# RikVoorhaar/tt-sketch

Hardware: AMD Instinct MI355X
Metric: TT-cores sketched/sec (fp64) + achieved MFMA % for d=6 n=200 r=50 stream_sketch (higher is better)
Workload: dtype f64

## Files before the change

tt_sketch_amd/csrc/chain_fused.h:

```cpp
#pragma once
#include "skinny.h"

namespace ttsk {

struct ChainStep {
    const double *W[SK_MAXB];
    const double *X[SK_MAXB];
    double *T[SK_MAXB];
    const double *E;
    double *slab;
    int nb, wpp, n;
    int K1, A, A2, J;
    int64_t w_c;
    int64_t x_j, x_k, x_c;
    int64_t x_extent, t_extent;
    int AP, A2P;
    int ebase;
    int eunits;
    int xcd_map;
    int diag;
    long long *stamps;
};

constexpr int CF_MAX_DMA = 160;

__device__ __forceinline__ void cf_barrier()
{
    asm volatile("s_waitcnt lgkmcnt(0)\n\ts_barrier" ::: "memory");
}
#ifdef TTSK_LAB
#define CF_DIAG(bit) (a.diag & (bit))
#define CF_STAMP(i) do { if (a.stamps && blockIdx.x == 0 && lane == 0 && k - k_beg < 8) a.stamps[((k - k_beg) * 8 + w) * 8 + (i)] = __builtin_amdgcn_s_memtime(); } while (0)
#else
#define CF_DIAG(bit) 0
#define CF_STAMP(i) do { } while (0)
#endif
#define CF_BARRIER() do { if (!CF_DIAG(4)) cf_barrier(); } while (0)

template <int NQF, int STRQ, int NNF, int STRN, int D, bool WT, int OCC, int EBUF, int UNR = 5 * D>
__global__ __launch_bounds__(512, 2 * OCC) void chain_step_kernel(ChainStep a)
{
    extern __shared__ double cf_lds[];
    double *Wl = cf_lds;
    double *El = cf_lds + a.ebase;
    const int tid = threadIdx.x, lane = tid & 63, w = tid >> 6;
    const int x16 = lane & 15, kq = lane >> 4;
    int prob, g;
    if (a.xcd_map) {
        const int gpx = a.wpp >> 3, xcd = blockIdx.x & 7, j = blockIdx.x >> 3;
        g = xcd * gpx + j % gpx;
        prob = j / gpx;
    } else {
        prob = blockIdx.x / a.wpp;
        g = blockIdx.x - prob * a.wpp;
    }
    const int k_beg = (int)((int64_t)g * a.n / a.wpp), k_end = (int)((int64_t)(g + 1) * a.n / a.wpp);
    const int NW = (a.J + 15) >> 4;
    const int KB1 = ((a.K1 + 3) / 4 + UNR - 1) / UNR * UNR;
    const int AP = a.AP, A2P = a.A2P;

    {
        const double *Wp = uniform_ptr(a.W[prob]);
        const __amdgpu_buffer_rsrc_t rw = make_rsrc(Wp, ((int64_t)(a.K1 - 1) * a.w_c + a.A) * 8);
        const int total = 4 * KB1 * AP;
        constexpr int BATCH = 10;
        for (int e0 = tid; e0 < total; e0 += 512 * BATCH) {
            double v[BATCH];
#pragma unroll
            for (int u = 0; u < BATCH; ++u) {
                const int e = e0 + 512 * u;
                const int c = e / AP, col = e - c * AP;
                v[u] = ld8(rw, (e < total && c < a.K1 && col < a.A) ? (uint32_t)(((int64_t)c * a.w_c + col) * 8) : OOB_OFF, 0);
            }
#pragma unroll
            for (int u = 0; u < BATCH; ++u) {
                const int e = e0 + 512 * u;
                const int c = e / AP, col = e - c * AP;
                if (e < total) Wl[(c >> 1) * 2 * AP + 2 * col + (c & 1)] = v[u];
            }
        }
    }

    if (w == 7) {
        const int NI = CF_DIAG(2) ? 0 : a.eunits >> 6;
        const uint32_t inv = (uint32_t)(((1ull << 32) + (uint32_t)A2P - 1) / (uint32_t)A2P);
        const int64_t rowstride = (int64_t)a.n * a.A2;
        const int ebuf = a.eunits * 2;
        auto fill = [&](int k) {
            const double *Ek = a.E + (int64_t)k * a.A2;
            double *dst = El + (EBUF == 2 ? (k & 1) * ebuf : 0);
#pragma unroll 2
            for (int m = 0; m < NI; ++m) {
                const uint32_t U = 64u * (uint32_t)m + (uint32_t)lane;
                const uint32_t sec = (uint32_t)(((uint64_t)U * inv) >> 32), u = U - sec * (uint32_t)A2P;
                int row = (int)(2 * sec + (u & 1));
                row = row < a.A ? row : a.A - 1;
                int col = (int)(2 * (u >> 1));
                col = col + 1 < a.A2 ? col : 0;
                __builtin_amdgcn_global_load_lds((const __attribute__((address_space(1))) void *)(Ek + row * rowstride + col),
                                                 (__attribute__((address_space(3))) void *)(dst + m * 128), 16, 0, 0);
            }
        };
        __syncthreads();
        if constexpr (EBUF == 2) {
            if (k_beg < k_end) fill(k_beg);
            for (int k = k_beg; k < k_end; ++k) {
                asm volatile("s_waitcnt vmcnt(0)" ::: "memory");
                CF_STAMP(1);
                CF_BARRIER();
                CF_STAMP(2);
                if (k + 1 < k_end) fill(k + 1);
                CF_STAMP(3);
                CF_BARRIER();
                CF_STAMP(4);
            }
        } else {
            for (int k = k_beg; k < k_end; ++k) {
                CF_STAMP(0);
                fill(k);
                asm volatile("s_waitcnt vmcnt(0)" ::: "memory");
                CF_STAMP(1);
                CF_BARRIER();
                CF_STAMP(2);
                CF_STAMP(3);
                CF_BARRIER();
                CF_STAMP(4);
            }
        }
        return;
    }
    __syncthreads();
    if (w >= NW) return;

    const int j0 = 16 * w;
    const bool jok = j0 + x16 < a.J;
    const uint32_t xlane = !CF_DIAG(1) ? (uint32_t)(((int64_t)(j0 + x16) * a.x_j + (int64_t)kq * a.x_c) * 8) : OOB_OFF;
    const __amdgpu_buffer_rsrc_t rx = make_rsrc(uniform_ptr(a.X[prob]), a.x_extent * 8);
    const uint32_t xstep = __builtin_amdgcn_readfirstlane((uint32_t)(4 * a.x_c * 8));
    const uint32_t kstep = __builtin_amdgcn_readfirstlane((uint32_t)(a.x_k * 8));
    static_assert(UNR % D == 0, "the unrolled body must keep the ring slots static");
    const int ITER = KB1 / UNR;
    auto xload = [&](uint32_t so) -> double { return ld8(rx, xlane, __builtin_amdgcn_readfirstlane(so)); };
    double ring[D];
#pragma unroll
    for (int d = 0; d < D; ++d) ring[d] = xload((uint32_t)k_beg * kstep + (uint32_t)d * xstep);

    v4d acc2[NNF ? NNF : 1];
    double acc2s[STRN ? STRN : 1];
#pragma unroll
    for (int p = 0; p < NNF; ++p)
#pragma unroll
        for (int t = 0; t < 4; ++t) acc2[p][t] = 0.0;
#pragma unroll
    for (int q = 0; q < STRN; ++q) acc2s[q] = 0.0;

    const int wl_lane = (kq >> 1) * 2 * AP + 2 * x16 + (kq & 1);
    const int ws_lane = (kq >> 1) * 2 * AP + 2 * (16 * NQF + (x16 & 3)) + (kq & 1);
    const int el_lane = (kq >> 1) * 2 * A2P + 4 * (x16 >> 1) + 2 * (kq & 1) + (x16 & 1);
    const int es_col = 16 * NNF + (x16 & 3);
    const int es_lane = (kq >> 1) * 2 * A2P + 2 * (kq & 1);

    __amdgpu_buffer_rsrc_t rt;
    if constexpr (WT) rt = make_rsrc(uniform_ptr(a.T[prob]), a.t_extent * 8);

    for (int k = k_beg; k < k_end; ++k) {
        v4d acc1[NQF ? NQF : 1];
        double acc1s[STRQ ? STRQ : 1];
#pragma unroll
        for (int p = 0; p < NQF; ++p)
#pragma unroll
            for (int t = 0; t < 4; ++t) acc1[p][t] = 0.0;
#pragma unroll
        for (int q = 0; q < STRQ; ++q) acc1s[q] = 0.0;

        CF_STAMP(0);
        double af[NQF ? NQF : 1], sf[STRQ ? STRQ : 1];
        auto wfetch = [&](const double *wrun, int u, double (&f)[NQF ? NQF : 1], double (&g)[STRQ ? STRQ : 1]) {
#pragma unroll
            for (int p = 0; p < NQF; ++p) f[p] = LDS_UNPAIRED(wrun[wl_lane + u * 4 * AP + 32 * p]);
#pragma unroll
            for (int q = 0; q < STRQ; ++q) g[q] = wrun[ws_lane + u * 4 * AP + 8 * q];
        };
        wfetch(Wl, 0, af, sf);
        uint32_t so = (uint32_t)k * kstep + (uint32_t)D * xstep;
        auto kblock = [&](const double *wrun, int u, bool wrap) {
            const int d = u % D;
            double afn[NQF ? NQF : 1], sfn[STRQ ? STRQ : 1];
            wfetch(wrun, u + 1, afn, sfn);
            const double bf = ring[d];
#pragma unroll
            for (int p = 0; p < NQF; ++p) acc1[p] = mfma16(af[p], bf, acc1[p]);
#pragma unroll
            for (int q = 0; q < STRQ; ++q) acc1s[q] = mfma4(sf[q], bf, acc1s[q]);
            if (wrap) so = (uint32_t)(k + 1) * kstep;
            ring[d] = xload(so);
            so += xstep;
#pragma unroll
            for (int p = 0; p < NQF; ++p) af[p] = afn[p];
#pragma unroll
            for (int q = 0; q < STRQ; ++q) sf[q] = sfn[q];
        };
        for (int it = 0; it < ITER; ++it) {
            const double *wrun = Wl + it * UNR * 4 * AP;
            const bool last = it == ITER - 1;
#pragma unroll
            for (int u = 0; u < UNR; ++u) kblock(wrun, u, last && u + D == UNR);
        }
        if constexpr (WT) {
            const int64_t nJ = (int64_t)a.n * a.J;
            const uint32_t tl = jok ? (uint32_t)(((int64_t)kq * nJ + (int64_t)k * a.J + j0 + x16) * 8) : OOB_OFF;
#pragma unroll
            for (int p = 0; p < NQF; ++p)
#pragma unroll
                for (int t = 0; t < 4; ++t)
                    st8(rt, (jok && 16 * p + 4 * t + kq < a.A) ? tl + (uint32_t)((16 * p + 4 * t) * nJ * 8) : OOB_OFF, acc1[p][t]);
#pragma unroll
            for (int q = 0; q < STRQ; ++q)
                st8(rt, (jok && 16 * NQF + 4 * q + kq < a.A) ? tl + (uint32_t)((16 * NQF + 4 * q) * nJ * 8) : OOB_OFF, acc1s[q]);
        }
        CF_STAMP(1);
        CF_BARRIER();
        CF_STAMP(2);

        {
            const double *eb = El + (EBUF == 2 ? (k & 1) * a.eunits * 2 : 0);
            double bf[NNF ? NNF : 1], bs[STRN ? STRN : 1];
            int el0 = el_lane, es0 = es_lane + 4 * (es_col >> 1) + (es_col & 1);
            asm volatile("" : "+v"(el0), "+v"(es0));
            auto efetch = [&](int kap, double (&f)[NNF ? NNF : 1], double (&g)[STRN ? STRN : 1]) {
#pragma unroll
                for (int nn = 0; nn < NNF; ++nn) f[nn] = LDS_UNPAIRED(eb[el0 + kap * 4 * A2P + 32 * nn]);
#pragma unroll
                for (int q = 0; q < STRN; ++q) g[q] = eb[es0 + kap * 4 * A2P + 8 * q];
            };
            double bf2[NNF ? NNF : 1], bs2[STRN ? STRN : 1];
            efetch(0, bf, bs);
            constexpr int KB2C = 4 * NQF + STRQ;
#pragma unroll
            for (int kap = 0; kap < KB2C; ++kap) {
                const int p = kap >> 2, t = kap & 3;
                const double af2 = p < NQF ? acc1[p < NQF ? p : 0][t] : acc1s[t < STRQ ? t : 0];
                if (kap & 1) {
                    if (kap + 1 < KB2C) efetch(kap + 1, bf, bs);
                    __builtin_amdgcn_sched_barrier(0);
#pragma unroll
                    for (int nn = 0; nn < NNF; ++nn) acc2[nn] = mfma16(af2, bf2[nn], acc2[nn]);
#pragma unroll
                    for (int q = 0; q < STRN; ++q) acc2s[q] = mfma4(af2, bs2[q], acc2s[q]);
                } else {
                    if (kap + 1 < KB2C) efetch(kap + 1, bf2, bs2);
                    __builtin_amdgcn_sched_barrier(0);
#pragma unroll
                    for (int nn = 0; nn < NNF; ++nn) acc2[nn] = mfma16(af2, bf[nn], acc2[nn]);
#pragma unroll
                    for (int q = 0; q < STRN; ++q) acc2s[q] = mfma4(af2, bs[q], acc2s[q]);
                }
            }
        }
        CF_STAMP(3);
        CF_BARRIER();
        CF_STAMP(4);
    }

    double *slab = a.slab + ((int64_t)prob * a.wpp + g) * a.J * a.A2;
#pragma unroll
    for (int nn = 0; nn < NNF; ++nn)
#pragma unroll
        for (int t = 0; t < 4; ++t) {
            const int j = j0 + 4 * t + kq, col = 16 * nn + x16;
            if (j < a.J && col < a.A2) slab[(int64_t)j * a.A2 + col] = acc2[nn][t];
        }
#pragma unroll
    for (int q = 0; q < STRN; ++q) {
        const int j = j0 + 4 * ((lane >> 2) & 3) + kq, col = 16 * NNF + 4 * q + (lane & 3);
        if (j < a.J && col < a.A2) slab[(int64_t)j * a.A2 + col] = acc2s[q];
    }
}

struct ChainStepArgs {
    int nb, n, K1, A, A2, J;
    const double *const *W;
    int64_t w_c;
    const double *const *X;
    int64_t x_j, x_k, x_c, x_extent;
    const double *E;
    double *const *T;
    double *const *Out;
};
int chain_fused_try(const ChainStepArgs &c, int stream, hipStream_t st, bool force = false);

}
```

tt_sketch_amd/csrc/chain_fused.hip:

```cpp
#include <cstdlib>
#include "chain_fused.h"

namespace ttsk {

int launch_chain_step_a(const ChainStep &a, int nf, int str, bool wt, int ebuf, int unr, size_t lds, int grid, hipStream_t st);
int launch_chain_step_b(const ChainStep &a, int nf, int str, bool wt, int ebuf, int unr, size_t lds, int grid, hipStream_t st);
int launch_chain_step_c(const ChainStep &a, int nf, int str, bool wt, int ebuf, int unr, size_t lds, int grid, hipStream_t st);
int launch_chain_step_d(const ChainStep &a, int nf, int str, bool wt, int ebuf, int unr, size_t lds, int grid, hipStream_t st);
int launch_chain_step_e(const ChainStep &a, int nf, int str, bool wt, int ebuf, int unr, size_t lds, int grid, hipStream_t st);

static int launch_chain_step(const ChainStep &a, int nf, int str, bool wt, int ebuf, int unr, size_t lds, int grid, hipStream_t st)
{
    if (nf <= 2) return launch_chain_step_a(a, nf, str, wt, ebuf, unr, lds, grid, st);
    if (nf <= 4) return launch_chain_step_b(a, nf, str, wt, ebuf, unr, lds, grid, st);
    if (nf == 5) return launch_chain_step_c(a, nf, str, wt, ebuf, unr, lds, grid, st);
    if (nf == 6) return launch_chain_step_d(a, nf, str, wt, ebuf, unr, lds, grid, st);
    return launch_chain_step_e(a, nf, str, wt, ebuf, unr, lds, grid, st);
}

static int cf_num_cu()
{
    static int n = [] {
        int dev = 0, v = 0;
        if (hipGetDevice(&dev) != hipSuccess) return 256;
        if (hipDeviceGetAttribute(&v, hipDeviceAttributeMultiprocessorCount, dev) != hipSuccess || v <= 0) return 256;
        return v;
    }();
    return n;
}

static void tile_split(int r, int &nf, int &str)
{
    const int rem = r % 16;
    nf = r / 16;
    if (rem == 0) str = 0;
    else if (rem <= 4) str = 1;
    else if (rem <= 8) str = 2;
    else { nf += 1; str = 0; }
}

// ... 19 lines not shown
    a.AP = 16 * nq + 4 * sq;
    a.A2P = c.A2;
    if (a.AP < 4 * KB2) return 0;
    const int64_t wl = (int64_t)4 * KB1 * a.AP;
    a.ebase = (int)((wl + 1) & ~(int64_t)1);
    const int64_t units = (int64_t)2 * KB2 * a.A2P;
    a.eunits = (int)cdiv(units, 64) * 64;
    if (a.eunits / 64 > CF_MAX_DMA) return 0;
    const int ebuf = nq <= 4 ? 2 : 1;
    const size_t lds = ((size_t)a.ebase + (size_t)a.eunits * 2 * ebuf) * 8;
    if (lds > 160 * 1024) return 0;
#ifdef TTSK_LAB
    { static int dg = [] { const char *e = getenv("TTSK_CF_DIAG"); return e ? atoi(e) : 0; }(); a.diag = dg; }
#endif
    if ((c.x_extent + c.x_k + 132 * c.x_c) * 8 >= (1ll << 32) - 64) return 0;
    if ((int64_t)c.A * c.n * c.A2 * 8 >= (1ll << 32) - 64) return 0;
    const bool wt = c.T != nullptr;
    a.t_extent = (int64_t)c.A * c.n * c.J;
    if (wt && (a.t_extent + (int64_t)16 * c.n * c.J) * 8 >= (1ll << 32) - 64) return 0;
    const int cus = cf_num_cu();
    int wpp = cus / c.nb > 0 ? cus / c.nb : 1;
    if (wpp > c.n) wpp = c.n;
    a.wpp = wpp;
    a.xcd_map = (wpp % 8 == 0 && wpp >= 8) ? 1 : 0;
    for (int b = 0; b < c.nb; ++b) {
        if ((uintptr_t)c.X[b] & 7) return 0;
        a.W[b] = c.W[b];
        a.X[b] = c.X[b];
        a.T[b] = wt ? c.T[b] : nullptr;
    }
    const int64_t nslab = (int64_t)c.nb * wpp;
    a.slab = (double *)scratch(stream, SCRATCH_GEMM, (size_t)nslab * c.J * c.A2 * 8 + 64);
    if (!a.slab) return TTSK_ERR_HIP;
    const bool prof = prof_on();
    if (prof) prof_open(st, 2.0 * c.nb * (double)c.n * c.J * ((double)c.K1 * c.A + (double)c.A * c.A2), 6,
                        nq * 100 + sq * 10 + (wt ? 1 : 0), unr == 25, false);
#ifdef TTSK_LAB
    static int stamps_on = [] { const char *e = getenv("TTSK_CF_STAMPS"); return e ? atoi(e) : 0; }();
#else
    constexpr int stamps_on = 0;
#endif
    long long *stamps_dev = nullptr;
    if (stamps_on) {
        if (hipMalloc(&stamps_dev, 8 * 8 * 8 * 8) != hipSuccess) return TTSK_ERR_HIP;
        (void)hipMemset(stamps_dev, 0, 8 * 8 * 8 * 8);
        a.stamps = stamps_dev;
    }
    int rc = launch_chain_step(a, nq, sq, wt, ebuf, unr, lds, (int)nslab, st);
    if (stamps_on) {
        long long h[8 * 8 * 8];
        (void)hipStreamSynchronize(st);
        (void)hipMemcpy(h, stamps_dev, sizeof(h), hipMemcpyDeviceToHost);
        (void)hipFree(stamps_dev);
        long long t0 = 0;
        for (int i = 0; i < 8 * 8 * 8; ++i) if (h[i] && (!t0 || h[i] < t0)) t0 = h[i];
        fprintf(stderr, "[cf stamps] workgroup 0: cycles since its first stamp; per slice, wave: start | endA | afterB1 | endB | afterB2\n");
        for (int sl = 0; sl < 4; ++sl)
            for (int w = 0; w < 8; ++w) {
                const long long *r = h + (sl * 8 + w) * 8;
                if (!r[1] && !r[4]) continue;
                fprintf(stderr, "  slice %d wave %d: %8lld %8lld %8lld %8lld %8lld\n", sl, w, r[0] ? r[0] - t0 : -1, r[1] - t0, r[2] - t0,
                        r[3] - t0, r[4] - t0);
            }
    }
    if (rc == TTSK_OK) {
        ReduceOut ro{};
        for (int b = 0; b < c.nb; ++b) ro.C[b] = c.Out[b];
        rc = launch_r_reduce(st, a.slab, wpp, c.J, c.A2, 1, (int64_t)c.J, ro, c.nb, (int64_t)c.A2, (int64_t)1, 1.0, 0);
    }
    if (prof) prof_close(st);
    return rc == TTSK_OK ? 1 : (rc == 1 ? 0 : rc);
}

}

using namespace ttsk;

extern "C" int ttsk_chain_step(int nb, int n, int K1, int A, int A2, int J, const double *const *W, int64_t w_c,
                               const double *const *X, int64_t x_j, int64_t x_k, int64_t x_c, int64_t x_extent,
                               const double *E, double *const *T, double *const *Out, int stream)
{
    TTSK_STREAM(st, stream);
// ... 11 lines not shown
```

tt_sketch_amd/csrc/chain_fused_ia.hip:

```cpp
#include "chain_fused_inst.h"

namespace ttsk {

int launch_chain_step_a(const ChainStep &a, int nf, int str, bool wt, int ebuf, int unr, size_t lds, int grid, hipStream_t st)
{
    TTSK_CF_CASE(1, 0, 2)
    TTSK_CF_CASE(1, 1, 2)
    TTSK_CF_CASE(1, 2, 2)
    TTSK_CF_CASE(2, 0, 2)
    TTSK_CF_CASE(2, 1, 2)
    TTSK_CF_CASE(2, 2, 2)
    return 1;
}

}
```

tt_sketch_amd/csrc/chain_fused_ib.hip:

```cpp
#include "chain_fused_inst.h"

namespace ttsk {

int launch_chain_step_b(const ChainStep &a, int nf, int str, bool wt, int ebuf, int unr, size_t lds, int grid, hipStream_t st)
{
    TTSK_CF_CASE(3, 0, 2)
    TTSK_CF_CASE(3, 1, 2)
    TTSK_CF_CASE(3, 2, 2)
    TTSK_CF_CASE(4, 0, 2)
    TTSK_CF_CASE(4, 1, 2)
    TTSK_CF_CASE(4, 2, 2)
    return 1;
}

}
```

tt_sketch_amd/csrc/chain_fused_ic.hip:

```cpp
#include "chain_fused_inst.h"

namespace ttsk {

int launch_chain_step_c(const ChainStep &a, int nf, int str, bool wt, int ebuf, int unr, size_t lds, int grid, hipStream_t st)
{
    TTSK_CF_CASE(5, 0, 1)
    TTSK_CF_CASE(5, 1, 1)
    TTSK_CF_CASE(5, 2, 1)
    return 1;
}

}
```

tt_sketch_amd/csrc/chain_fused_id.hip:

```cpp
#include "chain_fused_inst.h"

namespace ttsk {

int launch_chain_step_d(const ChainStep &a, int nf, int str, bool wt, int ebuf, int unr, size_t lds, int grid, hipStream_t st)
{
    TTSK_CF_CASE(6, 0, 1)
    TTSK_CF_CASE(6, 1, 1)
    TTSK_CF_CASE(6, 2, 1)
    return 1;
}

}
```

tt_sketch_amd/csrc/chain_fused_ie.hip:

```cpp
#include "chain_fused_inst.h"

namespace ttsk {

int launch_chain_step_e(const ChainStep &a, int nf, int str, bool wt, int ebuf, int unr, size_t lds, int grid, hipStream_t st)
{
    TTSK_CF_CASE(7, 0, 1)
    return 1;
}

}
```

tt_sketch_amd/csrc/chain_fused_inst.h:

```cpp
#pragma once
#include "chain_fused.h"

namespace ttsk {

#define TTSK_CF_KERN(NF, STR, WT, EBUF, UNR) chain_step_kernel<NF, STR, NF, STR, 5, WT, 1, EBUF, UNR>
#define TTSK_CF_CASE(NF, STR, EBUF)                                                                          \
    if (nf == NF && str == STR && ebuf == EBUF)                                                              \
        return launch(unr == 25 ? (wt ? TTSK_CF_KERN(NF, STR, true, EBUF, 25) : TTSK_CF_KERN(NF, STR, false, EBUF, 25)) \
                                : (wt ? TTSK_CF_KERN(NF, STR, true, EBUF, 5) : TTSK_CF_KERN(NF, STR, false, EBUF, 5)),   \
                      grid, 512, lds, st, a);

}
```

Measured before the change: 55420.

## Deal chain-step tiles across 12 waves with split and narrow-row pieces

Adds a host-side planner that splits the J tiles into pieces (whole tiles, tiles cut along the A dimension into two halves, and a 4-row variant for narrow trailing tiles) and assigns them to up to 12 waves, greedily balancing MFMA cycles across the four SIMDs. The kernel gains a 12-wave instantiation that dispatches each wave to its piece. Split halves combine their partial slab results through a block barrier and a read-modify-write. Spare waves are marked as load slots. The aim is to remove SIMD imbalance when the tile count does not map evenly onto 4 SIMDs, at the cost of lower occupancy (launch bounds of 1 block), extra barriers and more register pressure.

```diff
diff --git a/tt_sketch_amd/csrc/chain_deal.h b/tt_sketch_amd/csrc/chain_deal.h
--- /dev/null
+++ b/tt_sketch_amd/csrc/chain_deal.h
@@ -0,0 +1,99 @@
+#pragma once
+
+namespace ttsk {
+
+constexpr int CD_WAVES = 12;
+constexpr int CD_MAXPIECE = CD_WAVES - 1;
+constexpr int CD_NQF_MIN = 2, CD_KB2_MAX = 25;
+enum ChainPieceKind { CD_NONE = 0, CD_WHOLE = 1, CD_FIRST = 2, CD_REST = 3, CD_ROWS4 = 4 };
+
+constexpr int cd_cut(int nqf) { return nqf - (nqf + 1) / 3; }
+
+struct ChainPiece {
+    int tile;
+    int q0, nq;
+    int kind;
+    int slot;
+    long long cycles;
+};
+
+struct ChainDeal {
+    int waves;
+    int npieces;
+    ChainPiece piece[CD_MAXPIECE];
+    long long simd[4];
+    double useful;
+    double cap() const
+    {
+        long long m = simd[0];
+        for (int s = 1; s < 4; ++s) m = simd[s] > m ? simd[s] : m;
+        return m > 0 ? useful / (4.0 * (double)m) : 0.0;
+    }
+};
+
+inline ChainDeal chain_deal(int J, int A, int A2, int NQF, int STRQ, int NNF, int STRN, int kb1, bool cut = true)
+{
+    (void)A; (void)A2;
+    const long long colB = 64ll * NNF + 16ll * STRN;
+    auto cost = [&](int nfull, int nstrip) {
+        return (long long)kb1 * (64ll * nfull + 16ll * nstrip) + (long long)(4 * nfull + nstrip) * colB;
+    };
+    const long long cW = cost(NQF, STRQ);
+    const long long cR = 16ll * (NQF + STRQ) * (kb1 + 4 * NNF + STRN);
+    const int H = cd_cut(NQF);
+    const int NW = (J + 15) / 16;
+    const bool narrow = J % 16 >= 1 && J % 16 <= 4;
+
+    ChainDeal best{};
+    best.waves = 8;
+    best.npieces = NW;
+    for (int w = 0; w < NW; ++w) {
+        best.piece[w] = ChainPiece{w, 0, NQF + STRQ, CD_WHOLE, w, cW};
+        best.simd[w & 3] += cW;
+    }
+    best.useful = (double)J / 16.0 * (double)cW;
+    if (!cut || NW <= 4 || NW > 7 || NQF < CD_NQF_MIN || 4 * NQF + STRQ > CD_KB2_MAX) return best;
+
+    long long best_max = 0;
+    for (int s = 0; s < 4; ++s) best_max = best.simd[s] > best_max ? best.simd[s] : best_max;
+    const int nfull = narrow ? NW - 1 : NW;
+    for (int ncut = 0; ncut <= nfull; ++ncut) {
+        if (nfull + ncut + (narrow ? 1 : 0) > CD_MAXPIECE) break;
+        if (ncut == 0 && !narrow) continue;
+        ChainDeal d{};
+        d.waves = CD_WAVES;
+        d.useful = best.useful;
+        int np = 0;
+        for (int t = 0; t < nfull - ncut; ++t) d.piece[np++] = ChainPiece{t, 0, NQF + STRQ, CD_WHOLE, -1, cW};
+        for (int t = nfull - ncut; t < nfull; ++t) d.piece[np++] = ChainPiece{t, 0, H, CD_FIRST, -1, cost(H, 0)};
+        for (int t = nfull - ncut; t < nfull; ++t)
+            d.piece[np++] = ChainPiece{t, H, NQF - H + STRQ, CD_REST, -1, cost(NQF - H, STRQ)};
+        if (narrow) d.piece[np++] = ChainPiece{NW - 1, 0, NQF + STRQ, CD_ROWS4, -1, cR};
+        d.npieces = np;
+        for (int i = 1; i < np; ++i)
+            for (int j = i; j > 0 && d.piece[j].cycles > d.piece[j - 1].cycles; --j) {
+                const ChainPiece tmp = d.piece[j];
+                d.piece[j] = d.piece[j - 1];
+                d.piece[j - 1] = tmp;
+            }
+        int used[4] = {0, 0, 0, 0};
+        const int room[4] = {3, 3, 3, 2};
+        for (int i = 0; i < np; ++i) {
+            int s = -1;
+            for (int c = 0; c < 4; ++c)
+                if (used[c] < room[c] && (s < 0 || d.simd[c] < d.simd[s])) s = c;
+            d.piece[i].slot = s + 4 * used[s];
+            used[s] += 1;
+            d.simd[s] += d.piece[i].cycles;
+        }
+        long long m = 0;
+        for (int s = 0; s < 4; ++s) m = d.simd[s] > m ? d.simd[s] : m;
+        if (m < best_max) {
+            best_max = m;
+            best = d;
+        }
+    }
+    return best;
+}
+
+}
diff --git a/tt_sketch_amd/csrc/chain_fused.h b/tt_sketch_amd/csrc/chain_fused.h
--- a/tt_sketch_amd/csrc/chain_fused.h
+++ b/tt_sketch_amd/csrc/chain_fused.h
@@ -1,4 +1,5 @@
 #pragma once
+#include "chain_deal.h"
 #include "skinny.h"
 
 namespace ttsk {
@@ -18,6 +19,8 @@
     int ebase;
     int eunits;
     int xcd_map;
+    unsigned int piece[CD_WAVES];
+    int nload;
     int diag;
     long long *stamps;
 };
@@ -30,21 +33,290 @@
 }
 #ifdef TTSK_LAB
 #define CF_DIAG(bit) (a.diag & (bit))
-#define CF_STAMP(i) do { if (a.stamps && blockIdx.x == 0 && lane == 0 && k - k_beg < 8) a.stamps[((k - k_beg) * 8 + w) * 8 + (i)] = __builtin_amdgcn_s_memtime(); } while (0)
+#define CF_STAMP(i) do { if (a.stamps && blockIdx.x == 0 && lane == 0 && k - k_beg < 8) a.stamps[((k - k_beg) * CD_WAVES + w) * 8 + (i)] = __builtin_amdgcn_s_memtime(); } while (0)
 #else
 #define CF_DIAG(bit) 0
 #define CF_STAMP(i) do { } while (0)
 #endif
 #define CF_BARRIER() do { if (!CF_DIAG(4)) cf_barrier(); } while (0)
 
-template <int NQF, int STRQ, int NNF, int STRN, int D, bool WT, int OCC, int EBUF, int UNR = 5 * D>
-__global__ __launch_bounds__(512, 2 * OCC) void chain_step_kernel(ChainStep a)
+template <int NQF, int STRQ, int NNF, int STRN, int D, bool WT, int EBUF, int UNR, int KIND, int APC = 0>
+__device__ __forceinline__ void cf_piece(const ChainStep &a, const double *Wl, const double *El, int tile, int q0, int prob,
+                                         int g, int k_beg, int k_end, int KB1, int w, int lane)
+{
+    const int x16 = lane & 15, kq = lane >> 4;
+    const int AP = APC ? APC : a.AP, A2P = a.A2P;
+    const int j0 = 16 * tile;
+    const bool jok = j0 + x16 < a.J;
+    const uint32_t xlane = !CF_DIAG(1) ? (uint32_t)(((int64_t)(j0 + x16) * a.x_j + (int64_t)kq * a.x_c) * 8) : OOB_OFF;
+    const __amdgpu_buffer_rsrc_t rx = make_rsrc(uniform_ptr(a.X[prob]), a.x_extent * 8);
+    const uint32_t xstep = __builtin_amdgcn_readfirstlane((uint32_t)(4 * a.x_c * 8));
+    const uint32_t kstep = __builtin_amdgcn_readfirstlane((uint32_t)(a.x_k * 8));
+    static_assert(UNR % D == 0, "the unrolled body must keep the ring slots static");
+    const int ITER = KB1 / UNR;
+    auto xload = [&](uint32_t so) -> double { return ld8(rx, xlane, __builtin_amdgcn_readfirstlane(so)); };
+    double ring[D];
+#pragma unroll
+    for (int d = 0; d < D; ++d) ring[d] = xload((uint32_t)k_beg * kstep + (uint32_t)d * xstep);
+
+    v4d acc2[NNF ? NNF : 1];
+    double acc2s[STRN ? STRN : 1];
+#pragma unroll
+    for (int p = 0; p < NNF; ++p)
+#pragma unroll
+        for (int t = 0; t < 4; ++t) acc2[p][t] = 0.0;
+#pragma unroll
+    for (int q = 0; q < STRN; ++q) acc2s[q] = 0.0;
+
+    const int wl_lane = (kq >> 1) * 2 * AP + 2 * (16 * q0 + x16) + (kq & 1);
+    const int ws_lane = (kq >> 1) * 2 * AP + 2 * (16 * (q0 + NQF) + (x16 & 3)) + (kq & 1);
+    const int el_lane = (kq >> 1) * 2 * A2P + 4 * (x16 >> 1) + 2 * (kq & 1) + (x16 & 1);
+    const int es_col = 16 * NNF + (x16 & 3);
+    const int es_lane = (kq >> 1) * 2 * A2P + 2 * (kq & 1);
+
+    __amdgpu_buffer_rsrc_t rt;
+    if constexpr (WT) rt = make_rsrc(uniform_ptr(a.T[prob]), a.t_extent * 8);
+
+    for (int k = k_beg; k < k_end; ++k) {
+        v4d acc1[NQF ? NQF : 1];
+        double acc1s[STRQ ? STRQ : 1];
+#pragma unroll
+        for (int p = 0; p < NQF; ++p)
+#pragma unroll
+            for (int t = 0; t < 4; ++t) acc1[p][t] = 0.0;
+#pragma unroll
+        for (int q = 0; q < STRQ; ++q) acc1s[q] = 0.0;
+
+        CF_STAMP(0);
+        double af[NQF ? NQF : 1], sf[STRQ ? STRQ : 1];
+        auto wfetch = [&](const double *wrun, int u, double (&f)[NQF ? NQF : 1], double (&g)[STRQ ? STRQ : 1]) {
+#pragma unroll
+            for (int p = 0; p < NQF; ++p) f[p] = LDS_UNPAIRED(wrun[wl_lane + u * 4 * AP + 32 * p]);
+#pragma unroll
+            for (int q = 0; q < STRQ; ++q) g[q] = wrun[ws_lane + u * 4 * AP + 8 * q];
+        };
+        wfetch(Wl, 0, af, sf);
+        uint32_t so = (uint32_t)k * kstep + (uint32_t)D * xstep;
+        auto kblock = [&](const double *wrun, int u, bool wrap) {
+            const int d = u % D;
+            double afn[NQF ? NQF : 1], sfn[STRQ ? STRQ : 1];
+            wfetch(wrun, u + 1, afn, sfn);
+            const double bf = ring[d];
+#pragma unroll
+            for (int p = 0; p < NQF; ++p) acc1[p] = mfma16(af[p], bf, acc1[p]);
+#pragma unroll
+            for (int q = 0; q < STRQ; ++q) acc1s[q] = mfma4(sf[q], bf, acc1s[q]);
+            if (wrap) so = (uint32_t)(k + 1) * kstep;
+            ring[d] = xload(so);
+            so += xstep;
+#pragma unroll
+            for (int p = 0; p < NQF; ++p) af[p] = afn[p];
+#pragma unroll
+            for (int q = 0; q < STRQ; ++q) sf[q] = sfn[q];
+        };
+        for (int it = 0; it < ITER; ++it) {
+            const double *wrun = Wl + it * UNR * 4 * AP;
+            const bool last = it == ITER - 1;
+#pragma unroll
+            for (int u = 0; u < UNR; ++u) kblock(wrun, u, last && u + D == UNR);
+        }
+        if constexpr (WT) {
+            const int64_t nJ = (int64_t)a.n * a.J;
+            const int a0 = 16 * q0;
+            const uint32_t tl = jok ? (uint32_t)(((int64_t)(a0 + kq) * nJ + (int64_t)k * a.J + j0 + x16) * 8) : OOB_OFF;
+#pragma unroll
+            for (int p = 0; p < NQF; ++p)
+#pragma unroll
+                for (int t = 0; t < 4; ++t)
+                    st8(rt, (jok && a0 + 16 * p + 4 * t + kq < a.A) ? tl + (uint32_t)((16 * p + 4 * t) * nJ * 8) : OOB_OFF, acc1[p][t]);
+#pragma unroll
+            for (int q = 0; q < STRQ; ++q)
+                st8(rt, (jok && a0 + 16 * NQF + 4 * q + kq < a.A) ? tl + (uint32_t)((16 * NQF + 4 * q) * nJ * 8) : OOB_OFF, acc1s[q]);
+        }
+        CF_STAMP(1);
+        CF_BARRIER();
+        CF_STAMP(2);
+
+        {
+            const double *eb = El + (EBUF == 2 ? (k & 1) * a.eunits * 2 : 0) + q0 * 16 * A2P;
+            double bf[NNF ? NNF : 1], bs[STRN ? STRN : 1];
+            int el0 = el_lane, es0 = es_lane + 4 * (es_col >> 1) + (es_col & 1);
+            asm volatile("" : "+v"(el0), "+v"(es0));
+            auto efetch = [&](int kap, double (&f)[NNF ? NNF : 1], double (&g)[STRN ? STRN : 1]) {
+#pragma unroll
+                for (int nn = 0; nn < NNF; ++nn) f[nn] = LDS_UNPAIRED(eb[el0 + kap * 4 * A2P + 32 * nn]);
+#pragma unroll
+                for (int q = 0; q < STRN; ++q) g[q] = eb[es0 + kap * 4 * A2P + 8 * q];
+            };
+            double bf2[NNF ? NNF : 1], bs2[STRN ? STRN : 1];
+            efetch(0, bf, bs);
+            constexpr int KB2C = 4 * NQF + STRQ;
+#pragma unroll
+            for (int kap = 0; kap < KB2C; ++kap) {
+                const int p = kap >> 2, t = kap & 3;
+                const double af2 = p < NQF ? acc1[p < NQF ? p : 0][t] : acc1s[t < STRQ ? t : 0];
+                if (kap & 1) {
+                    if (kap + 1 < KB2C) efetch(kap + 1, bf, bs);
+                    __builtin_amdgcn_sched_barrier(0);
+#pragma unroll
+                    for (int nn = 0; nn < NNF; ++nn) acc2[nn] = mfma16(af2, bf2[nn], acc2[nn]);
+#pragma unroll
+                    for (int q = 0; q < STRN; ++q) acc2s[q] = mfma4(af2, bs2[q], acc2s[q]);
+                } else {
+                    if (kap + 1 < KB2C) efetch(kap + 1, bf2, bs2);
+                    __builtin_amdgcn_sched_barrier(0);
+#pragma unroll
+                    for (int nn = 0; nn < NNF; ++nn) acc2[nn] = mfma16(af2, bf[nn], acc2[nn]);
+#pragma unroll
+                    for (int q = 0; q < STRN; ++q) acc2s[q] = mfma4(af2, bs[q], acc2s[q]);
+                }
+            }
+        }
+        CF_STAMP(3);
+        CF_BARRIER();
+        CF_STAMP(4);
+    }
+
+    double *slab = a.slab + ((int64_t)prob * a.wpp + g) * a.J * a.A2;
+    if constexpr (KIND == CD_FIRST) __syncthreads();
+    int ln = lane;
+    if constexpr (APC != 0) asm volatile("v_mbcnt_lo_u32_b32 %0, -1, 0\n\tv_mbcnt_hi_u32_b32 %0, -1, %0" : "=v"(ln));
+    const int sx = ln & 15, sk = ln >> 4;
+#pragma unroll
+    for (int nn = 0; nn < NNF; ++nn)
+#pragma unroll
+        for (int t = 0; t < 4; ++t) {
+            const int j = j0 + 4 * t + sk, col = 16 * nn + sx;
+            if (j < a.J && col < a.A2) {
+                double *p = slab + (int64_t)j * a.A2 + col;
+                *p = KIND == CD_FIRST ? acc2[nn][t] + *p : acc2[nn][t];
+            }
+        }
+#pragma unroll
+    for (int q = 0; q < STRN; ++q) {
+        const int j = j0 + 4 * ((ln >> 2) & 3) + sk, col = 16 * NNF + 4 * q + (ln & 3);
+        if (j < a.J && col < a.A2) {
+            double *p = slab + (int64_t)j * a.A2 + col;
+            *p = KIND == CD_FIRST ? acc2s[q] + *p : acc2s[q];
+        }
+    }
+    if constexpr (KIND == CD_REST) {
+        __threadfence_block();
+        __syncthreads();
+    }
+}
+
+template <int NQF, int STRQ, int NNF, int STRN, int D, bool WT, int EBUF, int UNR, int APC>
+__device__ __forceinline__ void cf_rows4(const ChainStep &a, const double *Wl, const double *El, int tile, int prob, int g,
+                                         int k_beg, int k_end, int KB1, int w, int lane)
+{
+    constexpr int NC = 4 * NNF + STRN;
+    __builtin_amdgcn_s_setprio(2);
+    const int x16 = lane & 15, kq = lane >> 4, n4 = x16 & 3, beta = x16 >> 2;
+    constexpr int AP = APC;
+    const int A2P = a.A2P;
+    const int j0 = 16 * tile;
+    const bool jok = j0 + n4 < a.J;
+    const uint32_t xlane = !CF_DIAG(1) ? (uint32_t)(((int64_t)(j0 + n4) * a.x_j + (int64_t)kq * a.x_c) * 8) : OOB_OFF;
+    const __amdgpu_buffer_rsrc_t rx = make_rsrc(uniform_ptr(a.X[prob]), a.x_extent * 8);
+    const uint32_t xstep = __builtin_amdgcn_readfirstlane((uint32_t)(4 * a.x_c * 8));
+    const uint32_t kstep = __builtin_amdgcn_readfirstlane((uint32_t)(a.x_k * 8));
+    const int ITER = KB1 / UNR;
+    auto xload = [&](uint32_t so) -> double { return ld8(rx, xlane, __builtin_amdgcn_readfirstlane(so)); };
+    double ring[D];
+#pragma unroll
+    for (int d = 0; d < D; ++d) ring[d] = xload((uint32_t)k_beg * kstep + (uint32_t)d * xstep);
+
+    double acc2[NC];
+#pragma unroll
+    for (int c = 0; c < NC; ++c) acc2[c] = 0.0;
+
+    const int wl_lane = (kq >> 1) * 2 * AP + 2 * x16 + (kq & 1);
+    const int ws_lane = (kq >> 1) * 2 * AP + 2 * (16 * NQF + n4) + (kq & 1);
+    const int el_lane = (2 * beta + (kq >> 1)) * 2 * A2P + 4 * (n4 >> 1) + 2 * (kq & 1) + (n4 & 1);
+    const int es_lane = (kq >> 1) * 2 * A2P + 4 * (n4 >> 1) + 2 * (kq & 1) + (n4 & 1);
+
+    __amdgpu_buffer_rsrc_t rt;
+    if constexpr (WT) rt = make_rsrc(uniform_ptr(a.T[prob]), a.t_extent * 8);
+
+    for (int k = k_beg; k < k_end; ++k) {
+        double acc1[NQF], acc1s[STRQ ? STRQ : 1];
+#pragma unroll
+        for (int p = 0; p < NQF; ++p) acc1[p] = 0.0;
+#pragma unroll
+        for (int q = 0; q < STRQ; ++q) acc1s[q] = 0.0;
+        CF_STAMP(0);
+        uint32_t so = (uint32_t)k * kstep + (uint32_t)D * xstep;
+        for (int it = 0; it < ITER; ++it) {
+            const double *wrun = Wl + it * UNR * 4 * AP;
+            const bool last = it == ITER - 1;
+#pragma unroll
+            for (int u = 0; u < UNR; ++u) {
+                const int d = u % D;
+                const double bf = ring[d];
+#pragma unroll
+                for (int p = 0; p < NQF; ++p) acc1[p] = mfma4(LDS_UNPAIRED(wrun[wl_lane + u * 4 * AP + 32 * p]), bf, acc1[p]);
+#pragma unroll
+                for (int q = 0; q < STRQ; ++q) acc1s[q] = mfma4(wrun[ws_lane + u * 4 * AP + 8 * q], bf, acc1s[q]);
+                if (last && u + D == UNR) so = (uint32_t)(k + 1) * kstep;
+                ring[d] = xload(so);
+                so += xstep;
+            }
+        }
+        if constexpr (WT) {
+            const int64_t nJ = (int64_t)a.n * a.J;
+            const uint32_t tl = (uint32_t)(((int64_t)kq * nJ + (int64_t)k * a.J + j0 + n4) * 8);
+#pragma unroll
+            for (int p = 0; p < NQF; ++p)
+                st8(rt, (jok && 16 * p + 4 * beta + kq < a.A) ? tl + (uint32_t)((16 * p + 4 * beta) * nJ * 8) : OOB_OFF, acc1[p]);
+#pragma unroll
+            for (int q = 0; q < STRQ; ++q)
+                st8(rt, (jok && beta == 0 && 16 * NQF + 4 * q + kq < a.A) ? tl + (uint32_t)((16 * NQF + 4 * q) * nJ * 8) : OOB_OFF,
+                    acc1s[q]);
+        }
+        CF_STAMP(1);
+        CF_BARRIER();
+        CF_STAMP(2);
+        {
+            const double *eb = El + (EBUF == 2 ? (k & 1) * a.eunits * 2 : 0);
+            int el0 = el_lane, es0 = es_lane;
+            asm volatile("" : "+v"(el0), "+v"(es0));
+#pragma unroll
+            for (int p = 0; p < NQF; ++p)
+#pragma unroll
+                for (int c = 0; c < NC; ++c) acc2[c] = mfma4(acc1[p], eb[el0 + p * 16 * A2P + 8 * c], acc2[c]);
+#pragma unroll
+            for (int q = 0; q < STRQ; ++q)
+#pragma unroll
+                for (int c = 0; c < NC; ++c) {
+                    const double e = eb[es0 + (8 * NQF + 2 * q) * 2 * A2P + 8 * c];
+                    acc2[c] = mfma4(acc1s[q], beta == 0 ? e : 0.0, acc2[c]);
+                }
+        }
+        CF_STAMP(3);
+        CF_BARRIER();
+        CF_STAMP(4);
+    }
+
+    double *slab = a.slab + ((int64_t)prob * a.wpp + g) * a.J * a.A2;
+#pragma unroll
+    for (int c = 0; c < NC; ++c) {
+        double v = acc2[c];
+        v += __shfl_xor(v, 4);
+        v += __shfl_xor(v, 8);
+        const int j = j0 + kq, col = 4 * c + n4;
+        if (beta == 0 && j < a.J && col < a.A2) slab[(int64_t)j * a.A2 + col] = v;
+    }
+}
+
+template <int NQF, int STRQ, int NNF, int STRN, int D, bool WT, int OCC, int EBUF, int UNR = 5 * D, int NWV = 8>
+__global__ __launch_bounds__(64 * NWV, NWV == 8 ? 2 * OCC : 1) void chain_step_kernel(ChainStep a)
 {
     extern __shared__ double cf_lds[];
     double *Wl = cf_lds;
     double *El = cf_lds + a.ebase;
     const int tid = threadIdx.x, lane = tid & 63, w = tid >> 6;
-    const int x16 = lane & 15, kq = lane >> 4;
+    constexpr int NT = 64 * NWV;
     int prob, g;
     if (a.xcd_map) {
         const int gpx = a.wpp >> 3, xcd = blockIdx.x & 7, j = blockIdx.x >> 3;
@@ -55,7 +327,6 @@
         g = blockIdx.x - prob * a.wpp;
     }
     const int k_beg = (int)((int64_t)g * a.n / a.wpp), k_end = (int)((int64_t)(g + 1) * a.n / a.wpp);
-    const int NW = (a.J + 15) >> 4;
     const int KB1 = ((a.K1 + 3) / 4 + UNR - 1) / UNR * UNR;
     const int AP = a.AP, A2P = a.A2P;
 
@@ -64,24 +335,32 @@
         const __amdgpu_buffer_rsrc_t rw = make_rsrc(Wp, ((int64_t)(a.K1 - 1) * a.w_c + a.A) * 8);
         const int total = 4 * KB1 * AP;
         constexpr int BATCH = 10;
-        for (int e0 = tid; e0 < total; e0 += 512 * BATCH) {
+        for (int e0 = tid; e0 < total; e0 += NT * BATCH) {
             double v[BATCH];
 #pragma unroll
             for (int u = 0; u < BATCH; ++u) {
-                const int e = e0 + 512 * u;
+                const int e = e0 + NT * u;
                 const int c = e / AP, col = e - c * AP;
                 v[u] = ld8(rw, (e < total && c < a.K1 && col < a.A) ? (uint32_t)(((int64_t)c * a.w_c + col) * 8) : OOB_OFF, 0);
             }
 #pragma unroll
             for (int u = 0; u < BATCH; ++u) {
-                const int e = e0 + 512 * u;
+                const int e = e0 + NT * u;
                 const int c = e / AP, col = e - c * AP;
                 if (e < total) Wl[(c >> 1) * 2 * AP + 2 * col + (c & 1)] = v[u];
             }
         }
     }
 
-    if (w == 7) {
+    unsigned pc = 0;
+    int li = 0, nl = 1;
+    if constexpr (NWV != 8) {
+        pc = a.piece[__builtin_amdgcn_readfirstlane(w)];
+        li = __builtin_amdgcn_readfirstlane((pc >> 8) & 255);
+        nl = a.nload;
+    }
+    if (NWV == 8 ? w == 7 : __builtin_amdgcn_readfirstlane(pc >> 16) == CD_NONE) {
+        if constexpr (NWV != 8) __builtin_amdgcn_s_setprio(3);
         const int NI = CF_DIAG(2) ? 0 : a.eunits >> 6;
         const uint32_t inv = (uint32_t)(((1ull << 32) + (uint32_t)A2P - 1) / (uint32_t)A2P);
         const int64_t rowstride = (int64_t)a.n * a.A2;
@@ -90,7 +369,7 @@
             const double *Ek = a.E + (int64_t)k * a.A2;
             double *dst = El + (EBUF == 2 ? (k & 1) * ebuf : 0);
 #pragma unroll 2
-            for (int m = 0; m < NI; ++m) {
+            for (int m = li; m < NI; m += nl) {
                 const uint32_t U = 64u * (uint32_t)m + (uint32_t)lane;
                 const uint32_t sec = (uint32_t)(((uint64_t)U * inv) >> 32), u = U - sec * (uint32_t)A2P;
                 int row = (int)(2 * sec + (u & 1));
@@ -130,150 +409,20 @@
         return;
     }
     __syncthreads();
-    if (w >= NW) return;
-
-    const int j0 = 16 * w;
-    const bool jok = j0 + x16 < a.J;
-    const uint32_t xlane = !CF_DIAG(1) ? (uint32_t)(((int64_t)(j0 + x16) * a.x_j + (int64_t)kq * a.x_c) * 8) : OOB_OFF;
-    const __amdgpu_buffer_rsrc_t rx = make_rsrc(uniform_ptr(a.X[prob]), a.x_extent * 8);
-    const uint32_t xstep = __builtin_amdgcn_readfirstlane((uint32_t)(4 * a.x_c * 8));
-    const uint32_t kstep = __builtin_amdgcn_readfirstlane((uint32_t)(a.x_k * 8));
-    static_assert(UNR % D == 0, "the unrolled body must keep the ring slots static");
-    const int ITER = KB1 / UNR;
-    auto xload = [&](uint32_t so) -> double { return ld8(rx, xlane, __builtin_amdgcn_readfirstlane(so)); };
-    double ring[D];
-#pragma unroll
-    for (int d = 0; d < D; ++d) ring[d] = xload((uint32_t)k_beg * kstep + (uint32_t)d * xstep);
-
-    v4d acc2[NNF ? NNF : 1];
-    double acc2s[STRN ? STRN : 1];
-#pragma unroll
-    for (int p = 0; p < NNF; ++p)
-#pragma unroll
-        for (int t = 0; t < 4; ++t) acc2[p][t] = 0.0;
-#pragma unroll
-    for (int q = 0; q < STRN; ++q) acc2s[q] = 0.0;
-
-    const int wl_lane = (kq >> 1) * 2 * AP + 2 * x16 + (kq & 1);
-    const int ws_lane = (kq >> 1) * 2 * AP + 2 * (16 * NQF + (x16 & 3)) + (kq & 1);
-    const int el_lane = (kq >> 1) * 2 * A2P + 4 * (x16 >> 1) + 2 * (kq & 1) + (x16 & 1);
-    const int es_col = 16 * NNF + (x16 & 3);
-    const int es_lane = (kq >> 1) * 2 * A2P + 2 * (kq & 1);
-
-    __amdgpu_buffer_rsrc_t rt;
-    if constexpr (WT) rt = make_rsrc(uniform_ptr(a.T[prob]), a.t_extent * 8);
-
-    for (int k = k_beg; k < k_end; ++k) {
-        v4d acc1[NQF ? NQF : 1];
-        double acc1s[STRQ ? STRQ : 1];
-#pragma unroll
-        for (int p = 0; p < NQF; ++p)
-#pragma unroll
-            for (int t = 0; t < 4; ++t) acc1[p][t] = 0.0;
-#pragma unroll
-        for (int q = 0; q < STRQ; ++q) acc1s[q] = 0.0;
-
-        CF_STAMP(0);
-        double af[NQF ? NQF : 1], sf[STRQ ? STRQ : 1];
-        auto wfetch = [&](const double *wrun, int u, double (&f)[NQF ? NQF : 1], double (&g)[STRQ ? STRQ : 1]) {
-#pragma unroll
-            for (int p = 0; p < NQF; ++p) f[p] = LDS_UNPAIRED(wrun[wl_lane + u * 4 * AP + 32 * p]);
-#pragma unroll
-            for (int q = 0; q < STRQ; ++q) g[q] = wrun[ws_lane + u * 4 * AP + 8 * q];
-        };
-        wfetch(Wl, 0, af, sf);
-        uint32_t so = (uint32_t)k * kstep + (uint32_t)D * xstep;
-        auto kblock = [&](const double *wrun, int u, bool wrap) {
-            const int d = u % D;
-            double afn[NQF ? NQF : 1], sfn[STRQ ? STRQ : 1];
-            wfetch(wrun, u + 1, afn, sfn);
-            const double bf = ring[d];
-#pragma unroll
-            for (int p = 0; p < NQF; ++p) acc1[p] = mfma16(af[p], bf, acc1[p]);
-#pragma unroll
-            for (int q = 0; q < STRQ; ++q) acc1s[q] = mfma4(sf[q], bf, acc1s[q]);
-            if (wrap) so = (uint32_t)(k + 1) * kstep;
-            ring[d] = xload(so);
-            so += xstep;
-#pragma unroll
-            for (int p = 0; p < NQF; ++p) af[p] = afn[p];
-#pragma unroll
-            for (int q = 0; q < STRQ; ++q) sf[q] = sfn[q];
-        };
-        for (int it = 0; it < ITER; ++it) {
-            const double *wrun = Wl + it * UNR * 4 * AP;
-            const bool last = it == ITER - 1;
-#pragma unroll
-            for (int u = 0; u < UNR; ++u) kblock(wrun, u, last && u + D == UNR);
-        }
-        if constexpr (WT) {
-            const int64_t nJ = (int64_t)a.n * a.J;
-            const uint32_t tl = jok ? (uint32_t)(((int64_t)kq * nJ + (int64_t)k * a.J + j0 + x16) * 8) : OOB_OFF;
-#pragma unroll
-            for (int p = 0; p < NQF; ++p)
-#pragma unroll
-                for (int t = 0; t < 4; ++t)
-                    st8(rt, (jok && 16 * p + 4 * t + kq < a.A) ? tl + (uint32_t)((16 * p + 4 * t) * nJ * 8) : OOB_OFF, acc1[p][t]);
-#pragma unroll
-            for (int q = 0; q < STRQ; ++q)
-                st8(rt, (jok && 16 * NQF + 4 * q + kq < a.A) ? tl + (uint32_t)((16 * NQF + 4 * q) * nJ * 8) : OOB_OFF, acc1s[q]);
-        }
-        CF_STAMP(1);
-        CF_BARRIER();
-        CF_STAMP(2);
-
-        {
-            const double *eb = El + (EBUF == 2 ? (k & 1) * a.eunits * 2 : 0);
-            double bf[NNF ? NNF : 1], bs[STRN ? STRN : 1];
-            int el0 = el_lane, es0 = es_lane + 4 * (es_col >> 1) + (es_col & 1);
-            asm volatile("" : "+v"(el0), "+v"(es0));
-            auto efetch = [&](int kap, double (&f)[NNF ? NNF : 1], double (&g)[STRN ? STRN : 1]) {
-#pragma unroll
-                for (int nn = 0; nn < NNF; ++nn) f[nn] = LDS_UNPAIRED(eb[el0 + kap * 4 * A2P + 32 * nn]);
-#pragma unroll
-                for (int q = 0; q < STRN; ++q) g[q] = eb[es0 + kap * 4 * A2P + 8 * q];
-            };
-            double bf2[NNF ? NNF : 1], bs2[STRN ? STRN : 1];
-            efetch(0, bf, bs);
-            constexpr int KB2C = 4 * NQF + STRQ;
-#pragma unroll
-            for (int kap = 0; kap < KB2C; ++kap) {
-                const int p = kap >> 2, t = kap & 3;
-                const double af2 = p < NQF ? acc1[p < NQF ? p : 0][t] : acc1s[t < STRQ ? t : 0];
-                if (kap & 1) {
-                    if (kap + 1 < KB2C) efetch(kap + 1, bf, bs);
-                    __builtin_amdgcn_sched_barrier(0);
-#pragma unroll
-                    for (int nn = 0; nn < NNF; ++nn) acc2[nn] = mfma16(af2, bf2[nn], acc2[nn]);
-#pragma unroll
-                    for (int q = 0; q < STRN; ++q) acc2s[q] = mfma4(af2, bs2[q], acc2s[q]);
-                } else {
-                    if (kap + 1 < KB2C) efetch(kap + 1, bf2, bs2);
-                    __builtin_amdgcn_sched_barrier(0);
-#pragma unroll
-                    for (int nn = 0; nn < NNF; ++nn) acc2[nn] = mfma16(af2, bf[nn], acc2[nn]);
-#pragma unroll
-                    for (int q = 0; q < STRN; ++q) acc2s[q] = mfma4(af2, bs[q], acc2s[q]);
-                }
-            }
-        }
-        CF_STAMP(3);
-        CF_BARRIER();
-        CF_STAMP(4);
-    }
-
-    double *slab = a.slab + ((int64_t)prob * a.wpp + g) * a.J * a.A2;
-#pragma unroll
-    for (int nn = 0; nn < NNF; ++nn)
-#pragma unroll
-        for (int t = 0; t < 4; ++t) {
-            const int j = j0 + 4 * t + kq, col = 16 * nn + x16;
-            if (j < a.J && col < a.A2) slab[(int64_t)j * a.A2 + col] = acc2[nn][t];
-        }
-#pragma unroll
-    for (int q = 0; q < STRN; ++q) {
-        const int j = j0 + 4 * ((lane >> 2) & 3) + kq, col = 16 * NNF + 4 * q + (lane & 3);
-        if (j < a.J && col < a.A2) slab[(int64_t)j * a.A2 + col] = acc2s[q];
+    if constexpr (NWV == 8) {
+        if (w >= (a.J + 15) >> 4) return;
+        cf_piece<NQF, STRQ, NNF, STRN, D, WT, EBUF, UNR, CD_WHOLE>(a, Wl, El, w, 0, prob, g, k_beg, k_end, KB1, w, lane);
+    } else {
+        const int kind = __builtin_amdgcn_readfirstlane(pc >> 16), tile = __builtin_amdgcn_readfirstlane(pc & 255);
+        constexpr int H = cd_cut(NQF), APC = 16 * NQF + 4 * STRQ;
+        if (kind == CD_WHOLE)
+            cf_piece<NQF, STRQ, NNF, STRN, D, WT, EBUF, UNR, CD_WHOLE, APC>(a, Wl, El, tile, 0, prob, g, k_beg, k_end, KB1, w, lane);
+        else if (kind == CD_FIRST)
+            cf_piece<H, 0, NNF, STRN, D, WT, EBUF, UNR, CD_FIRST, APC>(a, Wl, El, tile, 0, prob, g, k_beg, k_end, KB1, w, lane);
+        else if (kind == CD_REST)
+            cf_piece<NQF - H, STRQ, NNF, STRN, D, WT, EBUF, UNR, CD_REST, APC>(a, Wl, El, tile, H, prob, g, k_beg, k_end, KB1, w, lane);
+        else if (kind == CD_ROWS4)
+            cf_rows4<NQF, STRQ, NNF, STRN, D, WT, EBUF, UNR, APC>(a, Wl, El, tile, prob, g, k_beg, k_end, KB1, w, lane);
     }
 }
 
diff --git a/tt_sketch_amd/csrc/chain_fused.hip b/tt_sketch_amd/csrc/chain_fused.hip
--- a/tt_sketch_amd/csrc/chain_fused.hip
+++ b/tt_sketch_amd/csrc/chain_fused.hip
@@ -3,19 +3,19 @@
 
 namespace ttsk {
 
-int launch_chain_step_a(const ChainStep &a, int nf, int str, bool wt, int ebuf, int unr, size_t lds, int grid, hipStream_t st);
-int launch_chain_step_b(const ChainStep &a, int nf, int str, bool wt, int ebuf, int unr, size_t lds, int grid, hipStream_t st);
-int launch_chain_step_c(const ChainStep &a, int nf, int str, bool wt, int ebuf, int unr, size_t lds, int grid, hipStream_t st);
-int launch_chain_step_d(const ChainStep &a, int nf, int str, bool wt, int ebuf, int unr, size_t lds, int grid, hipStream_t st);
-int launch_chain_step_e(const ChainStep &a, int nf, int str, bool wt, int ebuf, int unr, size_t lds, int grid, hipStream_t st);
+int launch_chain_step_a(const ChainStep &a, int nf, int str, bool wt, int ebuf, int unr, int waves, size_t lds, int grid, hipStream_t st);
+int launch_chain_step_b(const ChainStep &a, int nf, int str, bool wt, int ebuf, int unr, int waves, size_t lds, int grid, hipStream_t st);
+int launch_chain_step_c(const ChainStep &a, int nf, int str, bool wt, int ebuf, int unr, int waves, size_t lds, int grid, hipStream_t st);
+int launch_chain_step_d(const ChainStep &a, int nf, int str, bool wt, int ebuf, int unr, int waves, size_t lds, int grid, hipStream_t st);
+int launch_chain_step_e(const ChainStep &a, int nf, int str, bool wt, int ebuf, int unr, int waves, size_t lds, int grid, hipStream_t st);
 
-static int launch_chain_step(const ChainStep &a, int nf, int str, bool wt, int ebuf, int unr, size_t lds, int grid, hipStream_t st)
+static int launch_chain_step(const ChainStep &a, int nf, int str, bool wt, int ebuf, int unr, int waves, size_t lds, int grid, hipStream_t st)
 {
-    if (nf <= 2) return launch_chain_step_a(a, nf, str, wt, ebuf, unr, lds, grid, st);
-    if (nf <= 4) return launch_chain_step_b(a, nf, str, wt, ebuf, unr, lds, grid, st);
-    if (nf == 5) return launch_chain_step_c(a, nf, str, wt, ebuf, unr, lds, grid, st);
-    if (nf == 6) return launch_chain_step_d(a, nf, str, wt, ebuf, unr, lds, grid, st);
-    return launch_chain_step_e(a, nf, str, wt, ebuf, unr, lds, grid, st);
+    if (nf <= 2) return launch_chain_step_a(a, nf, str, wt, ebuf, unr, waves, lds, grid, st);
+    if (nf <= 4) return launch_chain_step_b(a, nf, str, wt, ebuf, unr, waves, lds, grid, st);
+    if (nf == 5) return launch_chain_step_c(a, nf, str, wt, ebuf, unr, waves, lds, grid, st);
+    if (nf == 6) return launch_chain_step_d(a, nf, str, wt, ebuf, unr, waves, lds, grid, st);
+    return launch_chain_step_e(a, nf, str, wt, ebuf, unr, waves, lds, grid, st);
 }
 
 static int cf_num_cu()
@@ -81,6 +81,17 @@
     int wpp = cus / c.nb > 0 ? cus / c.nb : 1;
     if (wpp > c.n) wpp = c.n;
     a.wpp = wpp;
+    const ChainDeal deal = chain_deal(c.J, c.A, c.A2, nq, sq, nn, sn, KB1, c.n >= 2 * wpp);
+    if (deal.waves == CD_WAVES) {
+        bool taken[CD_WAVES] = {};
+        for (int i = 0; i < deal.npieces; ++i) taken[deal.piece[i].slot] = true;
+        for (int s = 0; s < CD_WAVES; ++s)
+            if (!taken[s]) a.piece[s] = (unsigned)a.nload++ << 8 | (unsigned)CD_NONE << 16;
+        for (int i = 0; i < deal.npieces; ++i) {
+            const ChainPiece &p = deal.piece[i];
+            a.piece[p.slot] = (unsigned)p.tile | (unsigned)p.q0 << 8 | (unsigned)p.kind << 16;
+        }
+    }
     a.xcd_map = (wpp % 8 == 0 && wpp >= 8) ? 1 : 0;
     for (int b = 0; b < c.nb; ++b) {
         if ((uintptr_t)c.X[b] & 7) return 0;
@@ -101,22 +112,22 @@
 #endif
     long long *stamps_dev = nullptr;
     if (stamps_on) {
-        if (hipMalloc(&stamps_dev, 8 * 8 * 8 * 8) != hipSuccess) return TTSK_ERR_HIP;
-        (void)hipMemset(stamps_dev, 0, 8 * 8 * 8 * 8);
+        if (hipMalloc(&stamps_dev, 8 * CD_WAVES * 8 * 8) != hipSuccess) return TTSK_ERR_HIP;
+        (void)hipMemset(stamps_dev, 0, 8 * CD_WAVES * 8 * 8);
         a.stamps = stamps_dev;
     }
-    int rc = launch_chain_step(a, nq, sq, wt, ebuf, unr, lds, (int)nslab, st);
+    int rc = launch_chain_step(a, nq, sq, wt, ebuf, unr, deal.waves, lds, (int)nslab, st);
     if (stamps_on) {
-        long long h[8 * 8 * 8];
+        long long h[8 * CD_WAVES * 8];
         (void)hipStreamSynchronize(st);
         (void)hipMemcpy(h, stamps_dev, sizeof(h), hipMemcpyDeviceToHost);
         (void)hipFree(stamps_dev);
         long long t0 = 0;
-        for (int i = 0; i < 8 * 8 * 8; ++i) if (h[i] && (!t0 || h[i] < t0)) t0 = h[i];
+        for (int i = 0; i < 8 * CD_WAVES * 8; ++i) if (h[i] && (!t0 || h[i] < t0)) t0 = h[i];
         fprintf(stderr, "[cf stamps] workgroup 0: cycles since its first stamp; per slice, wave: start | endA | afterB1 | endB | afterB2\n");
         for (int sl = 0; sl < 4; ++sl)
-            for (int w = 0; w < 8; ++w) {
-                const long long *r = h + (sl * 8 + w) * 8;
+            for (int w = 0; w < CD_WAVES; ++w) {
+                const long long *r = h + (sl * CD_WAVES + w) * 8;
                 if (!r[1] && !r[4]) continue;
                 fprintf(stderr, "  slice %d wave %d: %8lld %8lld %8lld %8lld %8lld\n", sl, w, r[0] ? r[0] - t0 : -1, r[1] - t0, r[2] - t0,
                         r[3] - t0, r[4] - t0);
diff --git a/tt_sketch_amd/csrc/chain_fused_ia.hip b/tt_sketch_amd/csrc/chain_fused_ia.hip
--- a/tt_sketch_amd/csrc/chain_fused_ia.hip
+++ b/tt_sketch_amd/csrc/chain_fused_ia.hip
@@ -2,7 +2,7 @@
 
 namespace ttsk {
 
-int launch_chain_step_a(const ChainStep &a, int nf, int str, bool wt, int ebuf, int unr, size_t lds, int grid, hipStream_t st)
+int launch_chain_step_a(const ChainStep &a, int nf, int str, bool wt, int ebuf, int unr, int waves, size_t lds, int grid, hipStream_t st)
 {
     TTSK_CF_CASE(1, 0, 2)
     TTSK_CF_CASE(1, 1, 2)
diff --git a/tt_sketch_amd/csrc/chain_fused_ib.hip b/tt_sketch_amd/csrc/chain_fused_ib.hip
--- a/tt_sketch_amd/csrc/chain_fused_ib.hip
+++ b/tt_sketch_amd/csrc/chain_fused_ib.hip
@@ -2,7 +2,7 @@
 
 namespace ttsk {
 
-int launch_chain_step_b(const ChainStep &a, int nf, int str, bool wt, int ebuf, int unr, size_t lds, int grid, hipStream_t st)
+int launch_chain_step_b(const ChainStep &a, int nf, int str, bool wt, int ebuf, int unr, int waves, size_t lds, int grid, hipStream_t st)
 {
     TTSK_CF_CASE(3, 0, 2)
     TTSK_CF_CASE(3, 1, 2)
diff --git a/tt_sketch_amd/csrc/chain_fused_ic.hip b/tt_sketch_amd/csrc/chain_fused_ic.hip
--- a/tt_sketch_amd/csrc/chain_fused_ic.hip
+++ b/tt_sketch_amd/csrc/chain_fused_ic.hip
@@ -2,7 +2,7 @@
 
 namespace ttsk {
 
-int launch_chain_step_c(const ChainStep &a, int nf, int str, bool wt, int ebuf, int unr, size_t lds, int grid, hipStream_t st)
+int launch_chain_step_c(const ChainStep &a, int nf, int str, bool wt, int ebuf, int unr, int waves, size_t lds, int grid, hipStream_t st)
 {
     TTSK_CF_CASE(5, 0, 1)
     TTSK_CF_CASE(5, 1, 1)
diff --git a/tt_sketch_amd/csrc/chain_fused_id.hip b/tt_sketch_amd/csrc/chain_fused_id.hip
--- a/tt_sketch_amd/csrc/chain_fused_id.hip
+++ b/tt_sketch_amd/csrc/chain_fused_id.hip
@@ -2,7 +2,7 @@
 
 namespace ttsk {
 
-int launch_chain_step_d(const ChainStep &a, int nf, int str, bool wt, int ebuf, int unr, size_t lds, int grid, hipStream_t st)
+int launch_chain_step_d(const ChainStep &a, int nf, int str, bool wt, int ebuf, int unr, int waves, size_t lds, int grid, hipStream_t st)
 {
     TTSK_CF_CASE(6, 0, 1)
     TTSK_CF_CASE(6, 1, 1)
diff --git a/tt_sketch_amd/csrc/chain_fused_ie.hip b/tt_sketch_amd/csrc/chain_fused_ie.hip
--- a/tt_sketch_amd/csrc/chain_fused_ie.hip
+++ b/tt_sketch_amd/csrc/chain_fused_ie.hip
@@ -2,7 +2,7 @@
 
 namespace ttsk {
 
-int launch_chain_step_e(const ChainStep &a, int nf, int str, bool wt, int ebuf, int unr, size_t lds, int grid, hipStream_t st)
+int launch_chain_step_e(const ChainStep &a, int nf, int str, bool wt, int ebuf, int unr, int waves, size_t lds, int grid, hipStream_t st)
 {
     TTSK_CF_CASE(7, 0, 1)
     return 1;
diff --git a/tt_sketch_amd/csrc/chain_fused_inst.h b/tt_sketch_amd/csrc/chain_fused_inst.h
--- a/tt_sketch_amd/csrc/chain_fused_inst.h
+++ b/tt_sketch_amd/csrc/chain_fused_inst.h
@@ -3,11 +3,15 @@
 
 namespace ttsk {
 
-#define TTSK_CF_KERN(NF, STR, WT, EBUF, UNR) chain_step_kernel<NF, STR, NF, STR, 5, WT, 1, EBUF, UNR>
+#define TTSK_CF_KERN(NF, STR, WT, EBUF, UNR, NWV) chain_step_kernel<NF, STR, NF, STR, 5, WT, 1, EBUF, UNR, NWV>
+#define TTSK_CF_PICK(NF, STR, EBUF, NWV)                                                                      \
+    (unr == 25 ? (wt ? TTSK_CF_KERN(NF, STR, true, EBUF, 25, NWV) : TTSK_CF_KERN(NF, STR, false, EBUF, 25, NWV)) \
+               : (wt ? TTSK_CF_KERN(NF, STR, true, EBUF, 5, NWV) : TTSK_CF_KERN(NF, STR, false, EBUF, 5, NWV)))
 #define TTSK_CF_CASE(NF, STR, EBUF)                                                                          \
-    if (nf == NF && str == STR && ebuf == EBUF)                                                              \
-        return launch(unr == 25 ? (wt ? TTSK_CF_KERN(NF, STR, true, EBUF, 25) : TTSK_CF_KERN(NF, STR, false, EBUF, 25)) \
-                                : (wt ? TTSK_CF_KERN(NF, STR, true, EBUF, 5) : TTSK_CF_KERN(NF, STR, false, EBUF, 5)),   \
-                      grid, 512, lds, st, a);
+    if (nf == NF && str == STR && ebuf == EBUF) {                                                            \
+        if constexpr (NF >= CD_NQF_MIN && 4 * NF + STR <= CD_KB2_MAX)                                        \
+            if (waves == CD_WAVES) return launch(TTSK_CF_PICK(NF, STR, EBUF, CD_WAVES), grid, 64 * CD_WAVES, lds, st, a); \
+        return launch(TTSK_CF_PICK(NF, STR, EBUF, 8), grid, 512, lds, st, a);                                \
+    }
 
 }
```

After: 58870 (median of 6 runs). +6.2%, better.
